# COMBINE-lab/salmon

Hardware: NVIDIA H100
Metric: EM iters/s (higher is better)
Workload: dtype f64

## Files before the change

### salmon_b200/csrc/em.cu

```cuda
#include <cooperative_groups.h>
#include <cub/cub.cuh>
#include <float.h>
#include <math.h>
#include <stdarg.h>
#include <string.h>

#include <algorithm>
#include <string>
#include <vector>

#include "common.cuh"
#include "em_internal.h"

#include "em_kernels.cuh"

namespace sb {

static const void* const K_PERSISTENT[2] = {(const void*)k_em_persistent<false>, (const void*)k_em_persistent<true>};
static const void* const K_PERSISTENT_MGPU[2] = {(const void*)k_em_persistent_mgpu<false>,
                                                 (const void*)k_em_persistent_mgpu<true>};
static void (*const K_P1[2])(EmArgs) = {k_em_p1<false>, k_em_p1<true>};
static void (*const K_P2[2])(EmArgs, uint32_t) = {k_em_p2<false>, k_em_p2<true>};
static void (*const K_P2_PARTIAL[2])(EmArgs) = {k_em_p2_partial<false>, k_em_p2_partial<true>};

// ... 473 lines not shown
  if (!c) return;
  cudaSetDevice(c->device);
  cudaDeviceSynchronize();
  for (void* p : c->x_opened) cudaIpcCloseMemHandle(p);
  cudaFree(c->x_block); cudaFree(c->d_peers); cudaFree(c->d_xfail);
  sb_em_comm_destroy(c);
  free_all(c);
  for (int i = 0; i < 4; ++i) cudaEventDestroy(c->ev[i]);
  cudaStreamDestroy(c->stream);
  delete c;
}

extern "C" int sb_em_set_option(sb_em_ctx* c, const char* key, int64_t value) {
  if (!c || !key) { set_error("null argument"); return SB_ERR_INVALID; }
  if (!strcmp(key, "variant")) c->variant = (int)value;
  else if (!strcmp(key, "blocks_per_sm")) { c->blocks_per_sm = (int)value; c->prepared = false; }
  else if (!strcmp(key, "sell_group_cm") || !strcmp(key, "sell_group_tm")) {
    if (value < 32 || value > (1 << 20) || (value & (value - 1))) { set_error("sell_group must be a power of two >= 32"); return SB_ERR_INVALID; }
    (key[11] == 'c' ? c->sell_group_cm : c->sell_group_tm) = (int)value; c->prepared = false;
  }
  else if (!strcmp(key, "push_pass")) { c->push_pass = (int)value; }
  else if (!strcmp(key, "sample_offset")) { c->sample_offset = (uint32_t)value; }
  else if (!strcmp(key, "rebalance")) { c->rebalance = (int)value; c->prepared = false; }
  else { set_error("unknown option '%s'", key); return SB_ERR_INVALID; }
  return SB_OK;
}

extern "C" int sb_em_get_info(sb_em_ctx* c, const char* key, int64_t* value) {
  if (!c || !key || !value) { set_error("null argument"); return SB_ERR_INVALID; }
  if (!c->prepared) { set_error("sb_em_get_info before sb_em_prepare"); return SB_ERR_STATE; }
  auto stream = [](const SellDev& m) { return (int64_t)m.n_cols * 32 * 10 + (int64_t)m.long_entries * 12; };
  if (!strcmp(key, "stream_bytes")) { *value = stream(c->cm) + stream(c->tm); return SB_OK; }
  if (!strcmp(key, "warps")) { *value = (int64_t)c->grid * (EM_THREADS / 32); return SB_OK; }
  if (!strcmp(key, "ring_cols")) { *value = (int64_t)EM_CH * EM_RING; return SB_OK; }
  const size_t n = strlen(key);
  const SellDev* m = nullptr;
  if (n > 3 && !strcmp(key + n - 3, "_cm")) m = &c->cm;
  else if (n > 3 && !strcmp(key + n - 3, "_tm")) m = &c->tm;
  const std::string k(key, m ? n - 3 : n);
  if (m && k == "stream_bytes") *value = stream(*m);
  else if (m && k == "sell_cols") *value = m->n_cols;
  else if (m && k == "long_rows") *value = m->n_long;
  else if (m && k == "long_entries") *value = (int64_t)m->long_entries;
  else if (m && k == "fallback_rows") *value = m->n_fallback;
  else { set_error("unknown info key '%s'", key); return SB_ERR_INVALID; }
  return SB_OK;
}

extern "C" int sb_em_upload(sb_em_ctx* c, const sb_eq_csr* eq, const double* projected,
                            const double* eff_len, const uint64_t* unique) {
  if (!c || !eq || !projected || !eff_len || !unique) { set_error("null argument"); return SB_ERR_INVALID; }
  if (eq->n_classes && (!eq->off || !eq->counts)) { set_error("null CSR arrays"); return SB_ERR_INVALID; }
  SB_CUDA(cudaSetDevice(c->device));
  const uint64_t C = eq->n_classes;
  const uint32_t M = eq->n_txps;
  const uint64_t nnz = C ? eq->off[C] : 0;
  if (M == 0) { set_error("no transcripts"); return SB_ERR_INVALID; }
  if (nnz >= 0xfffffff0ull || C >= 0xfffffff0ull) {
    set_error("eq-class table too large for 32-bit device offsets (nnz=%llu)", (unsigned long long)nnz);
    return SB_ERR_INVALID;
  }
  if (nnz && (!eq->tids || !eq->weights)) { set_error("null CSR arrays"); return SB_ERR_INVALID; }
  c->C = C; c->M = M; c->nnz = nnz;
  c->prepared = false;
  SB_TRY(dev_alloc(&c->d_off, C + 1));
  SB_TRY(dev_alloc(&c->d_tids, nnz));
  SB_TRY(dev_alloc(&c->d_aux, nnz));
// ... 113 lines not shown
    });
    for (uint32_t i = 0; i < m.n_long; ++i) {
      if (h[3 * ord[i] + 2] - h[3 * ord[i] + 1] > LWARP) m.n_block = i + 1;
      m.long_entries += h[3 * i + 2] - h[3 * i + 1];
    }
    std::vector<uint32_t> h2(h.size());
    for (uint32_t i = 0; i < m.n_long; ++i)
      for (int k = 0; k < 3; ++k) h2[3 * i + k] = h[3 * ord[i] + k];
    SB_CUDA(cudaMemcpyAsync(m.long_rows, h2.data(), h2.size() * 4, cudaMemcpyHostToDevice, st));
    SB_CUDA(cudaStreamSynchronize(st));
  }
  k_warp_ranges<<<nblk(n_warps + 1, 256), 256, 0, st>>>(m.n_slices, m.slice_ptr, overhead, n_warps, m.warp_begin);
  c->launches++;
  return SB_OK;
}

static int em_rebalance(sb_em_ctx* c);

extern "C" int sb_em_prepare(sb_em_ctx* c, const sb_em_params* p, sb_em_stats* stats) {
  if (!c || !p) { set_error("null argument"); return SB_ERR_INVALID; }
  if (!c->uploaded) { set_error("sb_em_prepare before sb_em_upload"); return SB_ERR_STATE; }
  SB_CUDA(cudaSetDevice(c->device));
  cudaStream_t st = c->stream;
  c->params = *p;
  c->launches = 0;
  const uint64_t C = c->C;
  const uint32_t M = c->M;
  const uint64_t nnz = c->nnz;
  const bool row_space = c->nranks <= 1 && !c->fused_loopback;
  SB_CUDA(cudaEventRecord(c->ev[0], st));

  int occ = 0;
  for (int v = 0; v < 2; ++v) {
    SB_CUDA(cudaFuncSetAttribute(K_PERSISTENT[v], cudaFuncAttributeMaxDynamicSharedMemorySize, (int)EM_SMEM));
    SB_CUDA(cudaFuncSetAttribute((const void*)K_P1[v], cudaFuncAttributeMaxDynamicSharedMemorySize, (int)EM_SMEM));
    SB_CUDA(cudaFuncSetAttribute((const void*)K_P2[v], cudaFuncAttributeMaxDynamicSharedMemorySize, (int)EM_SMEM));
    SB_CUDA(cudaFuncSetAttribute((const void*)K_P2_PARTIAL[v], cudaFuncAttributeMaxDynamicSharedMemorySize, (int)EM_SMEM));
    SB_CUDA(cudaFuncSetAttribute(K_PERSISTENT_MGPU[v], cudaFuncAttributeMaxDynamicSharedMemorySize, (int)EM_SMEM));
  }
  const int vb = p->use_vbem ? 1 : 0;
  SB_CUDA(cudaOccupancyMaxActiveBlocksPerMultiprocessor(&occ, (c->nranks > 1 || c->fused_loopback) ? K_PERSISTENT_MGPU[vb] : K_PERSISTENT[vb],
                                                        EM_THREADS, EM_SMEM));
  if (occ < 1) { set_error("persistent EM kernel does not fit on an SM"); return SB_ERR_CUDA; }
  if (c->blocks_per_sm > 0) occ = std::min(occ, c->blocks_per_sm);
  c->grid = (uint32_t)(occ * c->n_sm);
  c->occ = occ;
  const uint32_t n_warps = c->grid * (EM_THREADS / 32);

  const uint64_t NP = std::max<uint64_t>(C, M) + 1;
  const uint64_t NS = std::max<uint64_t>(std::max<uint64_t>(C, nnz), (uint64_t)M) + 1;
  SB_TRY(dev_alloc(&c->d_efflens, M));
  SB_TRY(dev_alloc(&c->d_prior, M));
  SB_TRY(dev_alloc(&c->d_alpha0, M));
  SB_TRY(dev_alloc(&c->d_alpha, M));
  SB_TRY(dev_alloc(&c->d_theta, (size_t)M + 4));
  SB_CUDA(cudaMemsetAsync(c->d_theta, 0, ((size_t)M + 4) * 8, st));
  SB_TRY(dev_alloc(&c->d_base, M));
  SB_TRY(dev_alloc(&c->d_cw, nnz));
  SB_TRY(dev_alloc(&c->d_packed, NP));
  SB_TRY(dev_alloc(&c->d_packed2, NP));
  SB_TRY(dev_alloc(&c->d_packed_scan, NP));
  SB_TRY(dev_alloc(&c->d_valid, C));
  SB_TRY(dev_alloc(&c->d_cls_map, C));
  SB_TRY(dev_alloc(&c->d_scalars, 64));
  SB_TRY(dev_alloc(&c->d_tcnt, M));
  SB_TRY(dev_alloc(&c->d_tid_row, M));
  SB_TRY(dev_alloc(&c->d_sort_keys, NS));
  SB_TRY(dev_alloc(&c->d_sort_vals, NS));
  SB_TRY(dev_alloc(&c->d_sort_keys2, NS));
  SB_TRY(dev_alloc(&c->d_sort_vals2, NS));
  SB_TRY(dev_alloc(&c->d_order, NS));
  SB_CUDA(cudaMemsetAsync(c->d_base, 0, (size_t)M * 8, st));
  SB_CUDA(cudaMemsetAsync(c->d_scalars, 0, 64 * 8, st));
  SB_CUDA(cudaMemsetAsync(c->d_tcnt, 0, (size_t)M * 4, st));
  SB_CUDA(cudaMemsetAsync(c->d_tid_row, 0xff, (size_t)M * 4, st));
// ... 85 lines not shown
  SB_CUDA(cudaMemsetAsync(c->r_theta, 0, ((size_t)R + 4) * 8, st));
  SB_TRY(dev_alloc(&c->r_prior, (size_t)R + 1));
  SB_TRY(dev_alloc(&c->r_base, (size_t)R + 1));
  SB_TRY(dev_alloc(&c->r_alpha0, (size_t)R + 1));
  SB_CUDA(cudaMemcpyAsync(c->t_off + R, &nnzm, 4, cudaMemcpyHostToDevice, st));
  k_rank_fill<<<nblk(M, 256), 256, 0, st>>>(M, c->d_tcnt, c->d_packed_scan, c->t_off, c->d_rank_tid,
                                             c->d_packed2);
  c->launches++;
  if (nnzm) {
    k_gather_csc<<<nblk(nnzm, 256), 256, 0, st>>>(nnzm, c->d_sort_vals2, c->d_ent_cls, c->m_w,
                                                   c->t_idx, c->t_w);
    c->launches++;
  }
  if (R) {
    k_bucket_key<<<nblk(R, 256), 256, 0, st>>>(R, nullptr, c->d_packed2, (uint32_t)c->sell_group_tm, c->d_sort_keys, c->d_sort_vals);
    c->launches++;
    SB_TRY(sort_pairs(c, R, 32));
    SB_CUDA(cudaMemcpyAsync(c->d_rowperm, c->d_sort_vals2, (size_t)R * 4, cudaMemcpyDeviceToDevice, st));
    k_row_fill<<<nblk(R, 256), 256, 0, st>>>(R, c->d_rowperm, c->d_rank_tid, c->d_prior, c->d_base,
                                              c->d_alpha0, c->d_row_tid, c->d_tid_row, c->r_prior,
                                              c->r_base, c->r_alpha0);
    c->launches++;
  }
  if (nnzm) {
    if (row_space) {
      k_remap<<<nblk(nnzm, 256), 256, 0, st>>>(nnzm, c->m_idx, c->d_tid_row, c->m_idx_state);
      c->launches++;
    } else {
      SB_CUDA(cudaMemcpyAsync(c->m_idx_state, c->m_idx, (size_t)nnzm * 4, cudaMemcpyDeviceToDevice, st));
    }
  }
  SB_TRY(build_sell(c, c->cm, Cm, nullptr, c->m_off, c->m_idx_state, c->m_w, row_space ? R : M, OVERHEAD_P1, n_warps));
  SB_TRY(build_sell(c, c->tm, R, c->d_rowperm, c->t_off, c->t_idx, c->t_w, Cm, overhead_tm(c), n_warps));

  double* d_sum0 = c->d_scalars + 16;
  double* d_inact = c->d_scalars + 17;
  k_sum1<<<1, 1024, 0, st>>>(M, c->d_alpha0, c->d_prior, c->d_tid_row, 0, d_sum0);
  k_sum1<<<1, 1024, 0, st>>>(M, c->d_base, c->d_prior, c->d_tid_row, 1, d_inact);
  c->launches += 2;
  SB_CUDA(cudaMemcpyAsync(&c->sum0, d_sum0, 8, cudaMemcpyDeviceToHost, st));
  SB_CUDA(cudaMemcpyAsync(&c->inactive_sum, d_inact, 8, cudaMemcpyDeviceToHost, st));
  SB_TRY(dev_alloc(&c->d_sum_partial, (size_t)2 * std::max<uint32_t>(c->grid, 4096)));
  SB_CUDA(cudaStreamSynchronize(st));
  c->prepared = true;
  c->rebalance_rounds_done = 0;
  if (c->variant == 1 && (c->nranks <= 1 || (c->peers_ready && c->M <= c->x_cap)) && p->max_iter > 0) {
    for (int r = 0; r < c->rebalance; ++r) {
      int rc = em_rebalance(c);
      if (rc != SB_OK) { c->prepared = false; return rc; }
          c->rebalance_rounds_done++;
    }
  }
  const uint32_t prep_launches = c->launches;
  SB_CUDA(cudaEventRecord(c->ev[1], st));
  SB_CUDA(cudaEventSynchronize(c->ev[1]));
  float ms = 0;
  cudaEventElapsedTime(&ms, c->ev[0], c->ev[1]);
  c->prepare_ms = ms;
  c->prepared = true;
  if (stats) {
    memset(stats, 0, sizeof(*stats));
    stats->n_degenerate = c->n_degenerate;
    stats->n_multi_classes = Cm;
    stats->nnz_multi = nnzm;
    stats->n_active_txps = R;
    stats->prepare_ms = ms;
    stats->gpu_launches = prep_launches;
  }
  return SB_OK;
}

static Sell sell_view(const SellDev& m) {
  Sell s;
  s.slice_ptr = m.slice_ptr; s.base = m.base; s.len = m.len; s.idx = m.idx; s.w = m.w; s.warp_begin = m.warp_begin;
  s.long_rows = m.long_rows; s.csr_idx = m.csr_idx; s.csr_w = m.csr_w;
  s.n_rows = m.n_rows; s.n_slices = m.n_slices; s.n_long = m.n_long;
  s.n_block = m.n_block;
  s.zero = m.zero;
  return s;
}

static void fill_args(sb_em_ctx* c, EmArgs& A, bool row_space) {
  memset(&A, 0, sizeof(A));
  A.cm = sell_view(c->cm);
  A.tm = sell_view(c->tm);
  const bool ov = c->ov_active;
  A.c_cnt = (ov && c->ov_cnt) ? c->ov_cnt : c->d_cnt; A.scale = c->d_scale;
  if (row_space) {
    A.alpha = c->r_alpha; A.theta = c->r_theta; A.prior = c->r_prior;
    A.base = (ov && c->ov_base_row) ? c->ov_base_row : c->r_base;
    A.row_tid = nullptr;
  } else {
    A.alpha = c->d_alpha; A.theta = c->d_theta; A.prior = c->d_prior; A.base = c->d_base;
    A.row_tid = c->d_row_tid;
    A.tid_row = c->d_tid_row;
  }
  A.sum_partial = c->d_sum_partial;
  A.maxrel = (unsigned long long*)(c->d_scalars + 24);
  A.inactive_sum = ov ? c->ov_inactive_sum : c->inactive_sum;
  A.sum0 = ov ? c->ov_sum0 : c->sum0;
  A.min_eq_w = ov ? c->ov_min_eq_w : DBL_MIN;
  A.first_bias = ov ? 0.0 : (c->params.use_vbem ? 0.0 : 1.0);
  A.tol = c->params.tol; A.min_iter = c->params.min_iter; A.max_iter = c->params.max_iter;
  A.out = (uint32_t*)(c->d_scalars + 32);
  A.lq = (unsigned int*)(c->d_scalars + 44);
  A.dbg = c->dbg_enabled ? c->d_dbg : nullptr;
  A.dbg_it = c->dbg_it;
}

#include <dlfcn.h>
namespace {
struct NcclUid { char b[128]; };
struct NcclFns {
  void* h = nullptr;
  int (*GetUniqueId)(void*) = nullptr;
  int (*CommInitRank)(void**, int, NcclUid, int) = nullptr;
  int (*AllReduce)(const void*, void*, size_t, int, int, void*, cudaStream_t) = nullptr;
  int (*AllGather)(const void*, void*, size_t, int, void*, cudaStream_t) = nullptr;
  int (*CommDestroy)(void*) = nullptr;
  const char* (*GetErrorString)(int) = nullptr;
};
NcclFns g_nccl;
int nccl_load() {
  if (g_nccl.h) return SB_OK;
  const char* names[] = {"libnccl.so.2", "libnccl.so", nullptr};
  void* h = nullptr;
  for (int i = 0; names[i] && !h; ++i) h = dlopen(names[i], RTLD_NOW | RTLD_GLOBAL);
  if (!h) { set_error("cannot dlopen libnccl.so.2: %s", dlerror()); return SB_ERR_NCCL; }
  g_nccl.GetUniqueId = (decltype(g_nccl.GetUniqueId))dlsym(h, "ncclGetUniqueId");
  g_nccl.CommInitRank = (decltype(g_nccl.CommInitRank))dlsym(h, "ncclCommInitRank");
  g_nccl.AllReduce = (decltype(g_nccl.AllReduce))dlsym(h, "ncclAllReduce");
  g_nccl.AllGather = (decltype(g_nccl.AllGather))dlsym(h, "ncclAllGather");
  g_nccl.CommDestroy = (decltype(g_nccl.CommDestroy))dlsym(h, "ncclCommDestroy");
  g_nccl.GetErrorString = (decltype(g_nccl.GetErrorString))dlsym(h, "ncclGetErrorString");
  if (!g_nccl.GetUniqueId || !g_nccl.CommInitRank || !g_nccl.AllReduce || !g_nccl.AllGather || !g_nccl.CommDestroy) {
    set_error("libnccl is missing required symbols");
    return SB_ERR_NCCL;
  }
  g_nccl.h = h;
  return SB_OK;
// ... 244 lines not shown
  const int vb = c->params.use_vbem ? 1 : 0;
  uint32_t launches = 0;
  SB_CUDA(cudaEventRecord(c->ev[0], st));
  double* d_sum0 = c->d_scalars + 16;
  const bool fused = multi_gpu && c->peers_ready && c->M <= c->x_cap && c->variant == 1;
  const bool ov = c->ov_active;
  if (multi_gpu) {
    double* theta0 = fused ? reinterpret_cast<double*>(c->x_block + XchgLayout(M, (uint32_t)c->nranks).off_theta()) : c->d_theta;
    k_theta0<<<nblk(M, 256), 256, 0, st>>>(M, c->params.use_vbem, c->d_alpha0, c->d_prior, d_sum0,
                                            c->d_alpha, theta0);
    ++launches;
  } else if (R) {
    k_theta0<<<nblk(R, 256), 256, 0, st>>>(R, c->params.use_vbem,
                                            (ov && c->ov_alpha0_row) ? c->ov_alpha0_row : c->r_alpha0,
                                            c->r_prior, ov ? c->d_scalars + 18 : d_sum0,
                                            c->r_alpha, c->r_theta);
    ++launches;
  }
  SB_CUDA(cudaMemsetAsync(c->d_scalars + 24, 0, 16 * 8, st));
  SB_CUDA(cudaMemsetAsync(c->d_scalars + 44, 0, 16, st));
  EmArgs A;
  fill_args(c, A, !multi_gpu);
  uint32_t out[4] = {0, 0, 0, 0};
  float loop_ms = 0;
  uint32_t loop_launches = 0;
  if (c->params.max_iter == 0 && c->params.min_iter == 0) {
  } else if (multi_gpu) {
    int r = fused ? em_run_multi_gpu_fused(c, A, out, &launches, &loop_launches, &loop_ms)
                  : em_run_multi_gpu(c, A, out, &launches, &loop_launches, &loop_ms);
    if (r != SB_OK) return r;
  } else if (c->variant == 1) {
    void* args[] = {(void*)&A};
    SB_CUDA(cudaEventRecord(c->ev[2], st));
    SB_CUDA(cudaLaunchCooperativeKernel(K_PERSISTENT[vb], dim3(c->grid), dim3(EM_THREADS), args, EM_SMEM, st));
    SB_CUDA(cudaEventRecord(c->ev[3], st));
    ++launches; ++loop_launches;
    SB_CUDA(cudaMemcpyAsync(out, A.out, 16, cudaMemcpyDeviceToHost, st));
    SB_CUDA(cudaStreamSynchronize(st));
    cudaEventElapsedTime(&loop_ms, c->ev[2], c->ev[3]);
  } else {
    uint32_t it = 0;
    bool converged = false;
    SB_CUDA(cudaEventRecord(c->ev[2], st));
    while (it < A.min_iter || (it < A.max_iter && !converged)) {
      k_reset_maxrel<<<1, 1, 0, st>>>(A.maxrel, it & 1u);
      K_P1[vb]<<<c->grid, EM_THREADS, EM_SMEM, st>>>(A);
      K_P2[vb]<<<c->grid, EM_THREADS, EM_SMEM, st>>>(A, it);
      launches += 3; loop_launches += 2;
      ++it;
      if (it >= A.min_iter) {
        unsigned long long mr = 0;
        SB_CUDA(cudaMemcpyAsync(&mr, A.maxrel + ((it - 1) & 1u), 8, cudaMemcpyDeviceToHost, st));
        SB_CUDA(cudaStreamSynchronize(st));
        double d;
        memcpy(&d, &mr, 8);
        converged = !(d > A.tol);
      }
    }
    SB_CUDA(cudaEventRecord(c->ev[3], st));
    SB_CUDA(cudaStreamSynchronize(st));
    cudaEventElapsedTime(&loop_ms, c->ev[2], c->ev[3]);
    out[0] = it; out[1] = converged; out[2] = (it - 1) & 1u;
  }
  c->iters = out[0];
  c->converged = out[1];
  if (out[0] > 0) {
    unsigned long long mr = 0;
// ... 185 lines not shown
```

### salmon_b200/csrc/em_internal.h

```cpp
#pragma once
#include <cuda_runtime.h>
#include <stdint.h>

#include <vector>

#include "../../include/salmon_b200.h"

namespace sb {

constexpr int SELL_GROUP = 1024;

struct SellDev {
  uint32_t n_rows = 0, n_slices = 0, n_cols = 0, n_long = 0, n_block = 0;
  uint32_t n_fallback = 0;
  uint64_t long_entries = 0;
  uint32_t zero = 0;
  uint32_t* slice_ptr = nullptr;
  uint32_t* width = nullptr;
  uint32_t* base = nullptr;
  uint16_t* len = nullptr;
  uint16_t* idx = nullptr;
  double* w = nullptr;
  uint32_t* warp_begin = nullptr;
  uint32_t* long_rows = nullptr;
  const uint32_t* csr_idx = nullptr;
  const double* csr_w = nullptr;
};

}

struct sb_em_ctx {
  int device = 0;
  int n_sm = 0;
  size_t l2_bytes = 0;
  cudaStream_t stream = nullptr;
  cudaEvent_t ev[4] = {nullptr, nullptr, nullptr, nullptr};

  int variant = 1;
  int blocks_per_sm = 0;
  int rebalance = 1;
  int occ = 0;
  int sell_group_cm = sb::SELL_GROUP, sell_group_tm = sb::SELL_GROUP;

  uint64_t C = 0, nnz = 0;
  uint32_t M = 0;
  double total_weight = 0.0;
  size_t h2d_bytes = 0;
  bool uploaded = false, prepared = false;
  sb_em_params params{};

  uint64_t* d_off = nullptr;
  uint32_t* d_tids = nullptr;
  double* d_aux = nullptr;
  uint64_t* d_counts = nullptr;
  double* d_projected = nullptr;
  double* d_eff_in = nullptr;
  uint64_t* d_unique = nullptr;

  double* d_efflens = nullptr;
  double* d_prior = nullptr;
  double* d_alpha0 = nullptr;
  double* d_alpha = nullptr;
  double* d_theta = nullptr;
  double* d_base = nullptr;
  uint32_t* d_tcnt = nullptr;
  uint32_t* d_tid_row = nullptr;
  uint32_t* d_row_tid = nullptr;
  double *r_alpha = nullptr, *r_theta = nullptr, *r_prior = nullptr, *r_base = nullptr,
         *r_alpha0 = nullptr;

  double* d_cw = nullptr;
  uint64_t* d_packed = nullptr;
  uint64_t* d_packed2 = nullptr;
  uint64_t* d_packed_scan = nullptr;
// ... 67 lines not shown
```

### salmon_b200/csrc/em_kernels.cuh

```cuda
#pragma once
#include <cooperative_groups.h>
#include <float.h>

#include "common.cuh"
#include "em_math.h"

namespace sb {
namespace cg = cooperative_groups;

constexpr uint32_t LMAX = 96;
constexpr uint32_t LWARP = 2048;
constexpr int EM_THREADS = 256;
constexpr int EM_CH = 8;
constexpr int EM_RING = 4;
constexpr int EM_MIN_BLOCKS = 2;
constexpr double DIGAMMA_MIN = 1e-10;
constexpr double MIN_EQ_W = DBL_MIN;
constexpr double ALPHA_CHECK_CUTOFF = 1e-2;
constexpr uint16_t LEN_LONG = 0xFFFFu;
constexpr uint16_t IDX_PAD = 0xFFFFu;
constexpr uint32_t DBG_ACCUMULATE = 0xFFFFFFFFu;
constexpr uint32_t DBG_SLOTS = 16;

struct Sell {
  const uint32_t* slice_ptr;
  const uint32_t* base;
  const uint16_t* len;
  const uint16_t* idx;
  const double* w;
  const uint32_t* warp_begin;
  const uint32_t* long_rows;
  const uint32_t* csr_idx;
  const double* csr_w;
  uint32_t n_rows, n_slices, n_long;
  uint32_t n_block;
  uint32_t zero;
};

struct EmArgs {
  Sell cm;
  Sell tm;
  const double* c_cnt;
  double* scale;
  double* alpha; double* theta; const double* prior; const double* base;
  const uint32_t* row_tid;
  const uint32_t* tid_row;
  double* part_out;
  double* sum_partial;
  unsigned long long* maxrel;
  double inactive_sum; double sum0;
  double tol;
  double min_eq_w;
  double first_bias;
  uint32_t min_iter, max_iter;
  uint32_t* out;
  unsigned long long* dbg;
  uint32_t dbg_it;
  unsigned int* lq;
  unsigned char* const* peers;
  uint32_t rank, nranks, M;
  uint32_t push_pass;
  unsigned long long epoch0;
  uint32_t* xfail;
};

constexpr uint32_t XAUX = 1024;
struct XchgLayout {
  uint32_t M, G, S;
  __host__ __device__ XchgLayout(uint32_t m, uint32_t g) : M(m), G(g), S((m + g - 1) / g) {}
// ... 3 lines not shown
  __host__ __device__ size_t off_llth() const { return (off_alpha() + (size_t)M * 8 + 15) & ~(size_t)15; }
  __host__ __device__ size_t off_llaux() const { return off_llth() + (size_t)M * 16; }
  __host__ __device__ size_t off_llrecv() const { return off_llaux() + (size_t)G * XAUX * 2 * 16; }
  __host__ __device__ size_t bytes() const { return off_llrecv() + (size_t)G * S * 16; }
};

__device__ __forceinline__ unsigned long long gtime_ns() {
  unsigned long long t;
  asm volatile("mov.u64 %0, %%globaltimer;" : "=l"(t));
  return t;
}

constexpr double SUM_FIXED = 1048576.0;
struct P2Acc {
  long long isum;
  double maxrel;
};
__device__ __forceinline__ long long warp_sum_ll(long long v) {
#pragma unroll
  for (int o = 16; o > 0; o >>= 1) v += __shfl_xor_sync(0xffffffffu, v, o);
  return v;
}
__device__ __forceinline__ long long block_sum_ll(long long v, double* scratch) {
  const int lane = threadIdx.x & 31, wid = threadIdx.x >> 5;
  const int nw = (blockDim.x + 31) >> 5;
  v = warp_sum_ll(v);
  __syncthreads();
  if (lane == 0) scratch[wid] = __longlong_as_double(v);
  __syncthreads();
  long long r = (lane < nw) ? __double_as_longlong(scratch[lane]) : 0ll;
  return warp_sum_ll(r);
}

struct __align__(128) WarpRing {
  double w[EM_RING][EM_CH * 32];
  uint16_t idx[EM_RING][EM_CH * 32];
};
constexpr int EM_WARPS = EM_THREADS / 32;
constexpr size_t EM_SMEM = sizeof(WarpRing) * EM_WARPS + EM_WARPS * EM_RING * 8 + 40 * 8;

struct WarpCtx {
  WarpRing* ring;
  uint64_t* bars;
  uint32_t phase_bits;
  double* scratch;
  uint64_t pol_stream;
  unsigned long long* dbg;
  unsigned long long* dbg_acc;
  unsigned long long t0;
};

__device__ __forceinline__ void warp_setup(WarpCtx& W, unsigned char* smem) {
  const uint32_t wid = threadIdx.x >> 5;
  W.ring = reinterpret_cast<WarpRing*>(smem) + wid;
  W.bars = reinterpret_cast<uint64_t*>(smem + sizeof(WarpRing) * EM_WARPS) + wid * EM_RING;
  W.scratch = reinterpret_cast<double*>(smem + sizeof(WarpRing) * EM_WARPS + EM_WARPS * EM_RING * 8);
  W.phase_bits = 0;
  W.dbg = nullptr;
  W.dbg_acc = nullptr;
  W.t0 = 0;
  W.pol_stream = l2_policy_evict_first();
  if ((threadIdx.x & 31u) == 0) {
#pragma unroll
    for (int s = 0; s < EM_RING; ++s) mbar_init(&W.bars[s], 1);
    mbar_fence_init();
  }
  __syncthreads();
}

struct RowOps {
  double x0, x1, x2, x3;
  uint32_t len;
};
template <int PHASE>
__device__ __forceinline__ RowOps load_ops(const EmArgs& A, const Sell& S, uint32_t row) {
  RowOps o;
  o.x0 = o.x1 = o.x2 = o.x3 = 0.0;
  o.len = LEN_LONG;
  if (row < S.n_rows) {
    o.len = __ldg(&S.len[row]);
    if (PHASE == 1) {
      o.x0 = __ldg(&A.c_cnt[row]);
    } else if (PHASE == 2) {
      o.x0 = A.theta[row];
      o.x1 = __ldg(&A.prior[row]);
      o.x2 = __ldg(&A.base[row]);
      o.x3 = A.alpha[row];
    } else {
      const uint32_t t = __ldg(&A.row_tid[row]);
      o.x0 = A.theta[t];
      o.x2 = __ldg(&A.base[t]);
      o.x3 = __longlong_as_double((long long)t);
    }
  }
  return o;
}

template <bool VBEM>
__device__ __forceinline__ double theta_of(double na, double ap, double logNorm) {
  if (VBEM) return (ap > DIGAMMA_MIN) ? exp_digamma_shifted(ap, logNorm) : 0.0;
  return na;
}

template <int PHASE, bool VBEM, class Deliver>
__device__ __forceinline__ void row_finish(const EmArgs& A, uint32_t row, const RowOps& o, double acc,
                                           double logNorm, double bias, P2Acc& pa, Deliver&& deliver) {
  if (o.len == LEN_LONG) return;
  if (PHASE == 1) {
    A.scale[row] = (acc <= A.min_eq_w) ? 0.0 : o.x0 / acc;
  } else if (PHASE == 2) {
    const double th = o.x0, pr = o.x1;
    double na = o.x2 + bias;
    if (th > 0.0) na = fma(th, acc, na);
    if (na > ALPHA_CHECK_CUTOFF) pa.maxrel = fmax(pa.maxrel, fabs(o.x3 - na) / na);
    A.alpha[row] = na;
    const double ap = na + pr;
    pa.isum += __double2ll_rn(ap * SUM_FIXED);
    A.theta[row] = theta_of<VBEM>(na, ap, logNorm);
  } else {
    const uint32_t t = (uint32_t)__double_as_longlong(o.x3);
    double na = o.x2;
    if (o.x0 > 0.0) na = fma(o.x0, acc, na);
    deliver(t, na);
  }
}

struct WarpRange {
  uint32_t s0, s1, cbeg, cend;
};
__device__ __forceinline__ WarpRange load_range(const Sell& S, uint32_t gwarp) {
  WarpRange r;
  r.s0 = __ldg(&S.warp_begin[gwarp]);
  r.s1 = __ldg(&S.warp_begin[gwarp + 1]);
  r.cbeg = __ldg(&S.slice_ptr[r.s0]);
  r.cend = __ldg(&S.slice_ptr[r.s1]);
  return r;
}
__device__ __forceinline__ void ring_issue(const Sell& S, WarpCtx& W, const WarpRange& R, uint32_t k) {
  if ((threadIdx.x & 31u) == 0) {
    const uint32_t c = R.cbeg + k * EM_CH;
    const uint32_t cols = min((uint32_t)EM_CH, R.cend - c);
    const int st = k % EM_RING;
    mbar_arrive_expect_tx(&W.bars[st], cols * 320u);
    bulk_g2s_hint(W.ring->w[st], S.w + (size_t)c * 32u, cols * 256u, &W.bars[st], W.pol_stream);
    bulk_g2s_hint(W.ring->idx[st], S.idx + (size_t)c * 32u, cols * 64u, &W.bars[st], W.pol_stream);
  }
}
__device__ __forceinline__ void ring_prefetch(const Sell& S, WarpCtx& W, const WarpRange& R) {
  const uint32_t nchunks = (R.cend - R.cbeg + EM_CH - 1) / EM_CH;
#pragma unroll
  for (int k = 0; k < EM_RING; ++k)
    if ((uint32_t)k < nchunks) ring_issue(S, W, R, k);
}
__device__ __forceinline__ void ring_drain(WarpCtx& W, const WarpRange& R) {
  const uint32_t nchunks = (R.cend - R.cbeg + EM_CH - 1) / EM_CH;
#pragma unroll
  for (int k = 0; k < EM_RING; ++k)
    if ((uint32_t)k < nchunks) mbar_wait(&W.bars[k], (W.phase_bits >> k) & 1u);
}

struct RingCols {
  static constexpr uint32_t RC = (uint32_t)(EM_CH * EM_RING);
  const Sell& S;
  WarpCtx& W;
  const WarpRange& R;
  uint32_t lane, nchunks;
  uint32_t done = 0, ready = 0;
  __device__ __forceinline__ void need(uint32_t c0, uint32_t c1) {
    for (; (done + 1u) * EM_CH <= c0; ++done) {
      __syncwarp();
      if (done + EM_RING < nchunks) ring_issue(S, W, R, done + EM_RING);
    }
    for (; ready * EM_CH < c1; ++ready) {
      const int st = ready % EM_RING;
      mbar_wait(&W.bars[st], (W.phase_bits >> st) & 1u);
      W.phase_bits ^= (1u << st);
    }
  }
  __device__ __forceinline__ uint32_t group_at(uint32_t c) const {
    const uint32_t p = (c % RC) * 32u + lane * 4u;
    return p >= RC * 32u ? p - RC * 32u : p;
  }
  __device__ __forceinline__ uint2 idx4(uint32_t c) const {
    return *reinterpret_cast<const uint2*>(&W.ring->idx[0][0] + group_at(c));
  }
  __device__ __forceinline__ double2 w4(uint32_t c, uint32_t j) const {
    return *reinterpret_cast<const double2*>(&W.ring->w[0][0] + group_at(c) + j);
  }
  __device__ __forceinline__ uint32_t idx1(uint32_t c) const { return (&W.ring->idx[0][0])[(c % RC) * 32u + lane]; }
  __device__ __forceinline__ double w1(uint32_t c) const { return (&W.ring->w[0][0])[(c % RC) * 32u + lane]; }
};
template <int PHASE, bool VBEM, class Deliver>
__device__ __forceinline__ void sell_rows(const EmArgs& A, const Sell& S, RingCols& cols, uint32_t s0,
                                          uint32_t s1, uint32_t cbeg, uint32_t cend, double logNorm, double bias,
                                          P2Acc& pa, Deliver&& deliver) {
  const double* gsrc = (PHASE == 1) ? A.theta : A.scale;
  constexpr bool GUARD = (PHASE == 1) && !VBEM;
  const uint32_t lane = threadIdx.x & 31u;
  auto slot = [&](uint32_t base, uint32_t u) { return u == IDX_PAD ? S.zero : base + u; };
  auto fma1 = [&](double& acc, double g, double w) {
    if (GUARD) {
      const double v = g * w;
      if (!isnan(v)) acc += v;
    } else {
      acc = fma(g, w, acc);
    }
  };
  struct Group {
    double g0, g1, g2, g3;
    double2 wa, wb;
  };
  auto group_load = [&](uint32_t c, uint32_t base) {
    const uint2 i2 = cols.idx4(c);
    Group q;
    q.g0 = gsrc[slot(base, i2.x & 0xFFFFu)];
    q.g1 = gsrc[slot(base, i2.x >> 16)];
    q.g2 = gsrc[slot(base, i2.y & 0xFFFFu)];
    q.g3 = gsrc[slot(base, i2.y >> 16)];
    q.wa = cols.w4(c, 0u);
    q.wb = cols.w4(c, 2u);
    return q;
  };
  auto group_fma = [&](double& acc, const Group& q) {
    fma1(acc, q.g0, q.wa.x); fma1(acc, q.g1, q.wa.y); fma1(acc, q.g2, q.wb.x); fma1(acc, q.g3, q.wb.y);
  };
  uint32_t sbase = s0;
// ... 19 lines not shown
      cols.need(c, c + 8);
      const Group qa = group_load(c, base);
      const Group qb = group_load(c + 4, base);
      group_fma(acc, qa);
      group_fma(acc, qb);
    }
    if (ng) {
      cols.need(c, c + 4);
      group_fma(acc, group_load(c, base));
      c += 4;
    }
    if (rem) {
      cols.need(c, c + rem);
      const double g0 = gsrc[slot(base, cols.idx1(c))];
      if (rem == 1) {
        fma1(acc, g0, cols.w1(c));
      } else if (rem == 2) {
        const double g1 = gsrc[slot(base, cols.idx1(c + 1))];
        fma1(acc, g0, cols.w1(c)); fma1(acc, g1, cols.w1(c + 1));
      } else {
        const double g1 = gsrc[slot(base, cols.idx1(c + 1))], g2 = gsrc[slot(base, cols.idx1(c + 2))];
        fma1(acc, g0, cols.w1(c)); fma1(acc, g1, cols.w1(c + 1)); fma1(acc, g2, cols.w1(c + 2));
      }
      c += rem;
    }
    row_finish<PHASE, VBEM>(A, s * 32u + lane, ops, acc, logNorm, bias, pa, deliver);
  }
}

struct Nothing {
  __device__ __forceinline__ void operator()() const {}
};

template <int PHASE, bool VBEM, bool DYNQ, class AfterHome, class Deliver>
__device__ __forceinline__ void run_phase(const EmArgs& A, WarpCtx& W, const WarpRange& R,
                                          uint32_t bid, uint32_t nblk, double logNorm, double bias,
                                          P2Acc& pa, AfterHome&& after_home, Deliver&& deliver) {
  static_assert(EM_CH >= 8 && EM_RING >= 2, "two groups in flight span at most two resident chunks");
  const Sell& S = (PHASE == 1) ? A.cm : A.tm;
  const double* gsrc = (PHASE == 1) ? A.theta : A.scale;
  constexpr bool GUARD = (PHASE == 1) && !VBEM;
  const uint32_t lane = threadIdx.x & 31u;
  if (R.s1 > R.s0 && R.cend > R.cbeg) {
    RingCols rc{S, W, R, lane, (R.cend - R.cbeg + EM_CH - 1) / EM_CH};
    sell_rows<PHASE, VBEM>(A, S, rc, R.s0, R.s1, R.cbeg, R.cend, logNorm, bias, pa, deliver);
  }
  unsigned long long* const dbg = W.dbg;
  if (dbg && lane == 0) dbg[PHASE == 1 ? 8 : 7] = gtime_ns();
  if (W.dbg_acc && lane == 0) *W.dbg_acc += gtime_ns() - W.t0;
  __syncwarp();
  after_home();
  for (uint32_t li = bid; li < S.n_block; li += nblk) {
    const uint32_t r = __ldg(&S.long_rows[3 * li]);
    const uint32_t b = __ldg(&S.long_rows[3 * li + 1]);
    const uint32_t e = __ldg(&S.long_rows[3 * li + 2]);
    double a0 = 0.0, a1 = 0.0;
    uint32_t k = b + threadIdx.x;
    for (; k + EM_THREADS < e; k += 2 * EM_THREADS) {
      const uint32_t i0 = __ldg(&S.csr_idx[k]), i1 = __ldg(&S.csr_idx[k + EM_THREADS]);
      double v0 = gsrc[i0] * __ldg(&S.csr_w[k]);
      double v1 = gsrc[i1] * __ldg(&S.csr_w[k + EM_THREADS]);
      if (GUARD) {
        if (isnan(v0)) v0 = 0.0;
        if (isnan(v1)) v1 = 0.0;
      }
      a0 += v0;
      a1 += v1;
    }
    if (k < e) {
      double v = gsrc[__ldg(&S.csr_idx[k])] * __ldg(&S.csr_w[k]);
      if (GUARD && isnan(v)) v = 0.0;
      a0 += v;
    }
    const double acc = block_reduce<false>(a0 + a1, W.scratch);
    if (threadIdx.x == 0) {
      RowOps o = load_ops<PHASE>(A, S, r);
      o.len = 0;
      row_finish<PHASE, VBEM>(A, r, o, acc, logNorm, bias, pa, deliver);
// ... 102 lines not shown
__device__ __forceinline__ void lag_lognorm_warp0(const EmArgs& A, uint32_t par, uint32_t nblk,
                                                  double* scratch) {
  if (threadIdx.x < 32) {
    const double* part = A.sum_partial + (size_t)(par ^ 1u) * nblk;
    long long acc = 0;
    for (uint32_t i = threadIdx.x; i < nblk; i += 32) acc += __double_as_longlong(__ldcg(&part[i]));
    acc = warp_sum_ll(acc);
    if (threadIdx.x == 0) scratch[33] = digamma_pos((double)acc / SUM_FIXED + A.inactive_sum);
  }
}

__device__ __forceinline__ void p2_finish(const EmArgs& A, double* scratch, P2Acc& pa,
                                          uint32_t par) {
  const long long bs = block_sum_ll(pa.isum, scratch);
  double bm = block_reduce<true>(pa.maxrel, scratch);
  if (threadIdx.x == 0) {
    A.sum_partial[(size_t)par * gridDim.x + blockIdx.x] = __longlong_as_double(bs);
    if (bm > 0.0) atomicMax(&A.maxrel[par], (unsigned long long)__double_as_longlong(bm));
  }
}

#define SB_DBG(slot)                                                        \
  if (A.dbg && it == A.dbg_it && (threadIdx.x & 31u) == 0) A.dbg[(size_t)gwarp * DBG_SLOTS + (slot)] = gtime_ns();
#define SB_ACC_BEGIN(var, sell_slot) \
  unsigned long long var = 0; \
  if (dbg_acc) { var = gtime_ns(); W.t0 = var; W.dbg_acc = &A.dbg[(size_t)gwarp * DBG_SLOTS + (sell_slot)]; }
#define SB_ACC_END(var, slot) \
  W.dbg_acc = nullptr; \
  if (dbg_acc && (threadIdx.x & 31u) == 0) A.dbg[(size_t)gwarp * DBG_SLOTS + (slot)] += gtime_ns() - var;

template <bool VBEM>
__global__ void __launch_bounds__(EM_THREADS, EM_MIN_BLOCKS) k_em_persistent(const __grid_constant__ EmArgs A) {
  extern __shared__ __align__(128) unsigned char smem[];
  WarpCtx W;
  warp_setup(W, smem);
  double* scratch = W.scratch;
  cg::grid_group grid = cg::this_grid();
  const uint32_t bid = blockIdx.x, nblk = gridDim.x;
  const uint32_t gwarp = bid * (EM_THREADS / 32) + (threadIdx.x >> 5);
  const WarpRange R1 = load_range(A.cm, gwarp);
  const WarpRange R2 = load_range(A.tm, gwarp);
  uint32_t it = 0;
  bool converged = false;
  double logNorm = VBEM ? digamma_pos(A.sum0) : 0.0;
  ring_prefetch(A.cm, W, R1);
  while (it < A.min_iter || (it < A.max_iter && !converged)) {
    const uint32_t par = it & 1u;
    const bool dbg_acc = A.dbg && A.dbg_it == DBG_ACCUMULATE && it > 0;
    if (bid == 0 && threadIdx.x == 0) A.maxrel[par] = 0ull;
    if (VBEM && it > 0) lag_lognorm_warp0(A, par, nblk, scratch);
    P2Acc pa{0ll, 0.0};
    SB_DBG(0)
    SB_ACC_BEGIN(t1, 3)
    W.dbg = (A.dbg && it == A.dbg_it) ? &A.dbg[(size_t)gwarp * DBG_SLOTS] : nullptr;
    run_phase<1, VBEM, true>(A, W, R1, bid, nblk, 0.0, 0.0, pa, [&] { ring_prefetch(A.tm, W, R2); }, NoDeliver{});
    SB_ACC_END(t1, 0)
    SB_DBG(1)
    grid.sync();
    SB_DBG(2)
    if (bid == 0 && threadIdx.x == 0) A.lq[0] = 0u;
    if (VBEM && it > 0) logNorm = scratch[33];
    const double bias = (it == 0) ? A.first_bias : 0.0;
    SB_DBG(3)
    SB_ACC_BEGIN(t2, 4)
    run_phase<2, VBEM, true>(A, W, R2, bid, nblk, logNorm, bias, pa, [&] { ring_prefetch(A.cm, W, R1); }, NoDeliver{});
    W.dbg = nullptr;
    SB_ACC_END(t2, 1)
    SB_DBG(4)
    p2_finish(A, scratch, pa, par);
    SB_DBG(5)
    grid.sync();
    SB_DBG(6)
    if (bid == 0 && threadIdx.x == 0) A.lq[1] = 0u;
    if (dbg_acc && (threadIdx.x & 31u) == 0) A.dbg[(size_t)gwarp * DBG_SLOTS + 2] += 1ull;
// ... 291 lines not shown
```

Baseline: 26620.

## Keep leading SELL slices resident in shared memory across EM iterations

The persistent EM kernel now reserves spare shared memory per warp and, once at kernel start, bulk-loads the first SELL columns of each warp's cm and tm ranges into it. Each iteration then processes those slices straight from shared memory, and only the remaining columns are streamed through a smaller ring buffer (3 stages instead of 4). This is meant to cut repeated global/L2 streaming of matrix data on every iteration, at the cost of a shallower prefetch ring and more shared memory per block, which is capped to keep two blocks per SM. An info query for resident bytes is also added.

New measurement: 27180, median of 6. +2.1%, better.

```diff
diff --git a/salmon_b200/csrc/em.cu b/salmon_b200/csrc/em.cu
--- a/salmon_b200/csrc/em.cu
+++ b/salmon_b200/csrc/em.cu
@@ -529,7 +529,36 @@
   auto stream = [](const SellDev& m) { return (int64_t)m.n_cols * 32 * 10 + (int64_t)m.long_entries * 12; };
   if (!strcmp(key, "stream_bytes")) { *value = stream(c->cm) + stream(c->tm); return SB_OK; }
   if (!strcmp(key, "warps")) { *value = (int64_t)c->grid * (EM_THREADS / 32); return SB_OK; }
-  if (!strcmp(key, "ring_cols")) { *value = (int64_t)EM_CH * EM_RING; return SB_OK; }
+  if (!strcmp(key, "ring_cols")) { *value = (int64_t)EM_CH * EM_RING_RES; return SB_OK; }
+  if (!strcmp(key, "resident_cols_cm")) { *value = c->res_cm; return SB_OK; }
+  if (!strcmp(key, "resident_cols_tm")) { *value = c->res_cm ? EM_RES_COLS : 0; return SB_OK; }
+  if (!strcmp(key, "resident_bytes")) {
+    if (c->res_cm == 0) { *value = 0; return SB_OK; }
+    const uint32_t n_warps = c->grid * (EM_THREADS / 32);
+    std::vector<uint32_t> sp[2], wb[2];
+    SB_CUDA(cudaSetDevice(c->device));
+    for (int l = 0; l < 2; ++l) {
+      const SellDev& m = l ? c->tm : c->cm;
+      sp[l].resize((size_t)m.n_slices + 1);
+      wb[l].resize((size_t)n_warps + 1);
+      SB_CUDA(cudaMemcpy(sp[l].data(), m.slice_ptr, sp[l].size() * 4, cudaMemcpyDeviceToHost));
+      SB_CUDA(cudaMemcpy(wb[l].data(), m.warp_begin, wb[l].size() * 4, cudaMemcpyDeviceToHost));
+    }
+    int64_t b = 0;
+    for (uint32_t w = 0; w < n_warps; ++w) {
+      uint32_t budget = c->res_cm;
+      for (int l = 0; l < 2; ++l) {
+        const uint32_t s0 = wb[l][w], s1 = wb[l][w + 1];
+        uint32_t k = 0;
+        while (k < 32 && s0 + k < s1 && sp[l][s0 + k + 1] - sp[l][s0] <= budget) ++k;
+        const uint32_t cols = sp[l][s0 + k] - sp[l][s0];
+        b += (int64_t)cols * 320;
+        budget = EM_RES_COLS - cols;
+      }
+    }
+    *value = b;
+    return SB_OK;
+  }
   const size_t n = strlen(key);
   const SellDev* m = nullptr;
   if (n > 3 && !strcmp(key + n - 3, "_cm")) m = &c->cm;
@@ -709,15 +738,16 @@
 
   int occ = 0;
   for (int v = 0; v < 2; ++v) {
-    SB_CUDA(cudaFuncSetAttribute(K_PERSISTENT[v], cudaFuncAttributeMaxDynamicSharedMemorySize, (int)EM_SMEM));
+    SB_CUDA(cudaFuncSetAttribute(K_PERSISTENT[v], cudaFuncAttributeMaxDynamicSharedMemorySize, (int)EM_SMEM_RES));
     SB_CUDA(cudaFuncSetAttribute((const void*)K_P1[v], cudaFuncAttributeMaxDynamicSharedMemorySize, (int)EM_SMEM));
     SB_CUDA(cudaFuncSetAttribute((const void*)K_P2[v], cudaFuncAttributeMaxDynamicSharedMemorySize, (int)EM_SMEM));
     SB_CUDA(cudaFuncSetAttribute((const void*)K_P2_PARTIAL[v], cudaFuncAttributeMaxDynamicSharedMemorySize, (int)EM_SMEM));
     SB_CUDA(cudaFuncSetAttribute(K_PERSISTENT_MGPU[v], cudaFuncAttributeMaxDynamicSharedMemorySize, (int)EM_SMEM));
   }
   const int vb = p->use_vbem ? 1 : 0;
-  SB_CUDA(cudaOccupancyMaxActiveBlocksPerMultiprocessor(&occ, (c->nranks > 1 || c->fused_loopback) ? K_PERSISTENT_MGPU[vb] : K_PERSISTENT[vb],
-                                                        EM_THREADS, EM_SMEM));
+  const bool mgpu_kernel = c->nranks > 1 || c->fused_loopback;
+  SB_CUDA(cudaOccupancyMaxActiveBlocksPerMultiprocessor(&occ, mgpu_kernel ? K_PERSISTENT_MGPU[vb] : K_PERSISTENT[vb],
+                                                        EM_THREADS, mgpu_kernel ? EM_SMEM : EM_SMEM_RES));
   if (occ < 1) { set_error("persistent EM kernel does not fit on an SM"); return SB_ERR_CUDA; }
   if (c->blocks_per_sm > 0) occ = std::min(occ, c->blocks_per_sm);
   c->grid = (uint32_t)(occ * c->n_sm);
@@ -869,6 +899,7 @@
   }
   SB_TRY(build_sell(c, c->cm, Cm, nullptr, c->m_off, c->m_idx_state, c->m_w, row_space ? R : M, OVERHEAD_P1, n_warps));
   SB_TRY(build_sell(c, c->tm, R, c->d_rowperm, c->t_off, c->t_idx, c->t_w, Cm, overhead_tm(c), n_warps));
+  c->res_cm = row_space ? EM_RES_COLS : 0u;
 
   double* d_sum0 = c->d_scalars + 16;
   double* d_inact = c->d_scalars + 17;
@@ -914,6 +945,7 @@
   s.n_rows = m.n_rows; s.n_slices = m.n_slices; s.n_long = m.n_long;
   s.n_block = m.n_block;
   s.zero = m.zero;
+  s.nres = 0;
   return s;
 }
 
@@ -943,6 +975,7 @@
   A.lq = (unsigned int*)(c->d_scalars + 44);
   A.dbg = c->dbg_enabled ? c->d_dbg : nullptr;
   A.dbg_it = c->dbg_it;
+  A.cm.nres = c->res_cm;
 }
 
 #include <dlfcn.h>
@@ -1253,7 +1286,7 @@
   } else if (c->variant == 1) {
     void* args[] = {(void*)&A};
     SB_CUDA(cudaEventRecord(c->ev[2], st));
-    SB_CUDA(cudaLaunchCooperativeKernel(K_PERSISTENT[vb], dim3(c->grid), dim3(EM_THREADS), args, EM_SMEM, st));
+    SB_CUDA(cudaLaunchCooperativeKernel(K_PERSISTENT[vb], dim3(c->grid), dim3(EM_THREADS), args, EM_SMEM_RES, st));
     SB_CUDA(cudaEventRecord(c->ev[3], st));
     ++launches; ++loop_launches;
     SB_CUDA(cudaMemcpyAsync(out, A.out, 16, cudaMemcpyDeviceToHost, st));
diff --git a/salmon_b200/csrc/em_internal.h b/salmon_b200/csrc/em_internal.h
--- a/salmon_b200/csrc/em_internal.h
+++ b/salmon_b200/csrc/em_internal.h
@@ -40,6 +40,7 @@
   int blocks_per_sm = 0;
   int rebalance = 1;
   int occ = 0;
+  uint32_t res_cm = 0;
   int sell_group_cm = sb::SELL_GROUP, sell_group_tm = sb::SELL_GROUP;
 
   uint64_t C = 0, nnz = 0;
diff --git a/salmon_b200/csrc/em_kernels.cuh b/salmon_b200/csrc/em_kernels.cuh
--- a/salmon_b200/csrc/em_kernels.cuh
+++ b/salmon_b200/csrc/em_kernels.cuh
@@ -14,6 +14,8 @@
 constexpr int EM_CH = 8;
 constexpr int EM_RING = 4;
 constexpr int EM_MIN_BLOCKS = 2;
+constexpr int EM_RING_RES = 3;
+constexpr size_t EM_SMEM_MAX = 115712;
 constexpr double DIGAMMA_MIN = 1e-10;
 constexpr double MIN_EQ_W = DBL_MIN;
 constexpr double ALPHA_CHECK_CUTOFF = 1e-2;
@@ -35,6 +37,7 @@
   uint32_t n_rows, n_slices, n_long;
   uint32_t n_block;
   uint32_t zero;
+  uint32_t nres;
 };
 
 struct EmArgs {
@@ -104,15 +107,23 @@
   return warp_sum_ll(r);
 }
 
-struct __align__(128) WarpRing {
-  double w[EM_RING][EM_CH * 32];
-  uint16_t idx[EM_RING][EM_CH * 32];
+template <int NR>
+struct __align__(128) WarpRingT {
+  double w[NR][EM_CH * 32];
+  uint16_t idx[NR][EM_CH * 32];
 };
 constexpr int EM_WARPS = EM_THREADS / 32;
-constexpr size_t EM_SMEM = sizeof(WarpRing) * EM_WARPS + EM_WARPS * EM_RING * 8 + 40 * 8;
-
-struct WarpCtx {
-  WarpRing* ring;
+template <int NR>
+constexpr size_t ring_smem() { return sizeof(WarpRingT<NR>) * EM_WARPS + EM_WARPS * NR * 8 + 40 * 8; }
+constexpr size_t EM_SMEM = ring_smem<EM_RING>();
+constexpr size_t EM_SMEM_RING_RES = ring_smem<EM_RING_RES>();
+constexpr uint32_t EM_RES_COLS = (uint32_t)((EM_SMEM_MAX - EM_SMEM_RING_RES - EM_WARPS * 8) / (EM_WARPS * 320));
+constexpr size_t EM_SMEM_RES = EM_SMEM_RING_RES + EM_WARPS * 8 + (size_t)EM_WARPS * EM_RES_COLS * 320;
+static_assert(EM_SMEM_RES <= EM_SMEM_MAX, "k_em_persistent must keep EM_MIN_BLOCKS blocks per SM");
+
+template <int NR>
+struct WarpCtxT {
+  WarpRingT<NR>* ring;
   uint64_t* bars;
   uint32_t phase_bits;
   double* scratch;
@@ -121,12 +132,14 @@
   unsigned long long* dbg_acc;
   unsigned long long t0;
 };
-
-__device__ __forceinline__ void warp_setup(WarpCtx& W, unsigned char* smem) {
+using WarpCtx = WarpCtxT<EM_RING>;
+
+template <int NR>
+__device__ __forceinline__ void warp_setup(WarpCtxT<NR>& W, unsigned char* smem) {
   const uint32_t wid = threadIdx.x >> 5;
-  W.ring = reinterpret_cast<WarpRing*>(smem) + wid;
-  W.bars = reinterpret_cast<uint64_t*>(smem + sizeof(WarpRing) * EM_WARPS) + wid * EM_RING;
-  W.scratch = reinterpret_cast<double*>(smem + sizeof(WarpRing) * EM_WARPS + EM_WARPS * EM_RING * 8);
+  W.ring = reinterpret_cast<WarpRingT<NR>*>(smem) + wid;
+  W.bars = reinterpret_cast<uint64_t*>(smem + sizeof(WarpRingT<NR>) * EM_WARPS) + wid * NR;
+  W.scratch = reinterpret_cast<double*>(smem + sizeof(WarpRingT<NR>) * EM_WARPS + EM_WARPS * NR * 8);
   W.phase_bits = 0;
   W.dbg = nullptr;
   W.dbg_acc = nullptr;
@@ -134,7 +147,7 @@
   W.pol_stream = l2_policy_evict_first();
   if ((threadIdx.x & 31u) == 0) {
 #pragma unroll
-    for (int s = 0; s < EM_RING; ++s) mbar_init(&W.bars[s], 1);
+    for (int s = 0; s < NR; ++s) mbar_init(&W.bars[s], 1);
     mbar_fence_init();
   }
   __syncthreads();
@@ -198,7 +211,9 @@
 }
 
 struct WarpRange {
+  static constexpr bool RESIDENT = false;
   uint32_t s0, s1, cbeg, cend;
+  __device__ __forceinline__ uint32_t sbeg() const { return cbeg; }
 };
 __device__ __forceinline__ WarpRange load_range(const Sell& S, uint32_t gwarp) {
   WarpRange r;
@@ -208,43 +223,91 @@
   r.cend = __ldg(&S.slice_ptr[r.s1]);
   return r;
 }
-__device__ __forceinline__ void ring_issue(const Sell& S, WarpCtx& W, const WarpRange& R, uint32_t k) {
+struct ResRange : WarpRange {
+  static constexpr bool RESIDENT = true;
+  uint32_t sres, nres;
+  const double* rw;
+  const uint16_t* ri;
+  __device__ __forceinline__ uint32_t sbeg() const { return cbeg + nres; }
+};
+__device__ __forceinline__ ResRange load_res_range(const Sell& S, uint32_t gwarp, uint32_t ncols, uint32_t off,
+                                                   unsigned char* smem) {
+  ResRange r;
+  static_cast<WarpRange&>(r) = load_range(S, gwarp);
+  const uint32_t lane = threadIdx.x & 31u;
+  const bool in = r.s0 + lane < r.s1;
+  const uint32_t end = in ? __ldg(&S.slice_ptr[r.s0 + lane + 1u]) : r.cend;
+  const uint32_t k = __popc(__ballot_sync(0xffffffffu, in && end - r.cbeg <= ncols));
+  r.sres = r.s0 + k;
+  r.nres = k ? __shfl_sync(0xffffffffu, end, (int)k - 1) - r.cbeg : 0u;
+  unsigned char* area = smem + EM_SMEM_RING_RES + EM_WARPS * 8 + (threadIdx.x >> 5) * (EM_RES_COLS * 320u);
+  r.rw = reinterpret_cast<const double*>(area) + off * 32u;
+  r.ri = reinterpret_cast<const uint16_t*>(area + EM_RES_COLS * 256u) + off * 32u;
+  return r;
+}
+__device__ __forceinline__ void res_load(const Sell& S1, const ResRange& R1, const Sell& S2, const ResRange& R2,
+                                         uint64_t pol, unsigned char* smem) {
+  uint64_t* bar = reinterpret_cast<uint64_t*>(smem + EM_SMEM_RING_RES) + (threadIdx.x >> 5);
+  const uint32_t bytes = (R1.nres + R2.nres) * 320u;
+  if (bytes == 0) return;
   if ((threadIdx.x & 31u) == 0) {
-    const uint32_t c = R.cbeg + k * EM_CH;
+    mbar_init(bar, 1);
+    mbar_fence_init();
+    mbar_arrive_expect_tx(bar, bytes);
+    if (R1.nres) {
+      bulk_g2s_hint(const_cast<double*>(R1.rw), S1.w + (size_t)R1.cbeg * 32u, R1.nres * 256u, bar, pol);
+      bulk_g2s_hint(const_cast<uint16_t*>(R1.ri), S1.idx + (size_t)R1.cbeg * 32u, R1.nres * 64u, bar, pol);
+    }
+    if (R2.nres) {
+      bulk_g2s_hint(const_cast<double*>(R2.rw), S2.w + (size_t)R2.cbeg * 32u, R2.nres * 256u, bar, pol);
+      bulk_g2s_hint(const_cast<uint16_t*>(R2.ri), S2.idx + (size_t)R2.cbeg * 32u, R2.nres * 64u, bar, pol);
+    }
+  }
+  __syncwarp();
+  mbar_wait(bar, 0u);
+}
+
+template <int NR, class Range>
+__device__ __forceinline__ void ring_issue(const Sell& S, WarpCtxT<NR>& W, const Range& R, uint32_t k) {
+  if ((threadIdx.x & 31u) == 0) {
+    const uint32_t c = R.sbeg() + k * EM_CH;
     const uint32_t cols = min((uint32_t)EM_CH, R.cend - c);
-    const int st = k % EM_RING;
+    const int st = k % NR;
     mbar_arrive_expect_tx(&W.bars[st], cols * 320u);
     bulk_g2s_hint(W.ring->w[st], S.w + (size_t)c * 32u, cols * 256u, &W.bars[st], W.pol_stream);
     bulk_g2s_hint(W.ring->idx[st], S.idx + (size_t)c * 32u, cols * 64u, &W.bars[st], W.pol_stream);
   }
 }
-__device__ __forceinline__ void ring_prefetch(const Sell& S, WarpCtx& W, const WarpRange& R) {
-  const uint32_t nchunks = (R.cend - R.cbeg + EM_CH - 1) / EM_CH;
+template <int NR, class Range>
+__device__ __forceinline__ void ring_prefetch(const Sell& S, WarpCtxT<NR>& W, const Range& R) {
+  const uint32_t nchunks = (R.cend - R.sbeg() + EM_CH - 1) / EM_CH;
 #pragma unroll
-  for (int k = 0; k < EM_RING; ++k)
+  for (int k = 0; k < NR; ++k)
     if ((uint32_t)k < nchunks) ring_issue(S, W, R, k);
 }
-__device__ __forceinline__ void ring_drain(WarpCtx& W, const WarpRange& R) {
-  const uint32_t nchunks = (R.cend - R.cbeg + EM_CH - 1) / EM_CH;
+template <int NR, class Range>
+__device__ __forceinline__ void ring_drain(WarpCtxT<NR>& W, const Range& R) {
+  const uint32_t nchunks = (R.cend - R.sbeg() + EM_CH - 1) / EM_CH;
 #pragma unroll
-  for (int k = 0; k < EM_RING; ++k)
+  for (int k = 0; k < NR; ++k)
     if ((uint32_t)k < nchunks) mbar_wait(&W.bars[k], (W.phase_bits >> k) & 1u);
 }
 
+template <int NR, class Range>
 struct RingCols {
-  static constexpr uint32_t RC = (uint32_t)(EM_CH * EM_RING);
+  static constexpr uint32_t RC = (uint32_t)(EM_CH * NR);
   const Sell& S;
-  WarpCtx& W;
-  const WarpRange& R;
+  WarpCtxT<NR>& W;
+  const Range& R;
   uint32_t lane, nchunks;
   uint32_t done = 0, ready = 0;
   __device__ __forceinline__ void need(uint32_t c0, uint32_t c1) {
     for (; (done + 1u) * EM_CH <= c0; ++done) {
       __syncwarp();
-      if (done + EM_RING < nchunks) ring_issue(S, W, R, done + EM_RING);
+      if (done + NR < nchunks) ring_issue(S, W, R, done + NR);
     }
     for (; ready * EM_CH < c1; ++ready) {
-      const int st = ready % EM_RING;
+      const int st = ready % NR;
       mbar_wait(&W.bars[st], (W.phase_bits >> st) & 1u);
       W.phase_bits ^= (1u << st);
     }
@@ -262,8 +325,22 @@
   __device__ __forceinline__ uint32_t idx1(uint32_t c) const { return (&W.ring->idx[0][0])[(c % RC) * 32u + lane]; }
   __device__ __forceinline__ double w1(uint32_t c) const { return (&W.ring->w[0][0])[(c % RC) * 32u + lane]; }
 };
-template <int PHASE, bool VBEM, class Deliver>
-__device__ __forceinline__ void sell_rows(const EmArgs& A, const Sell& S, RingCols& cols, uint32_t s0,
+struct ResCols {
+  const double* w;
+  const uint16_t* idx;
+  uint32_t lane;
+  __device__ __forceinline__ void need(uint32_t, uint32_t) const {}
+  __device__ __forceinline__ uint2 idx4(uint32_t c) const {
+    return *reinterpret_cast<const uint2*>(idx + c * 32u + lane * 4u);
+  }
+  __device__ __forceinline__ double2 w4(uint32_t c, uint32_t j) const {
+    return *reinterpret_cast<const double2*>(w + c * 32u + lane * 4u + j);
+  }
+  __device__ __forceinline__ uint32_t idx1(uint32_t c) const { return idx[c * 32u + lane]; }
+  __device__ __forceinline__ double w1(uint32_t c) const { return w[c * 32u + lane]; }
+};
+template <int PHASE, bool VBEM, class Cols, class Deliver>
+__device__ __forceinline__ void sell_rows(const EmArgs& A, const Sell& S, Cols& cols, uint32_t s0,
                                           uint32_t s1, uint32_t cbeg, uint32_t cend, double logNorm, double bias,
                                           P2Acc& pa, Deliver&& deliver) {
   const double* gsrc = (PHASE == 1) ? A.theta : A.scale;
@@ -349,18 +426,28 @@
   __device__ __forceinline__ void operator()() const {}
 };
 
-template <int PHASE, bool VBEM, bool DYNQ, class AfterHome, class Deliver>
-__device__ __forceinline__ void run_phase(const EmArgs& A, WarpCtx& W, const WarpRange& R,
+template <int PHASE, bool VBEM, bool DYNQ, int NR, class Range, class AfterHome, class Deliver>
+__device__ __forceinline__ void run_phase(const EmArgs& A, WarpCtxT<NR>& W, const Range& R,
                                           uint32_t bid, uint32_t nblk, double logNorm, double bias,
                                           P2Acc& pa, AfterHome&& after_home, Deliver&& deliver) {
-  static_assert(EM_CH >= 8 && EM_RING >= 2, "two groups in flight span at most two resident chunks");
+  static_assert(EM_CH >= 8 && NR >= 2, "two groups in flight span at most two resident chunks");
   const Sell& S = (PHASE == 1) ? A.cm : A.tm;
   const double* gsrc = (PHASE == 1) ? A.theta : A.scale;
   constexpr bool GUARD = (PHASE == 1) && !VBEM;
   const uint32_t lane = threadIdx.x & 31u;
   if (R.s1 > R.s0 && R.cend > R.cbeg) {
-    RingCols rc{S, W, R, lane, (R.cend - R.cbeg + EM_CH - 1) / EM_CH};
-    sell_rows<PHASE, VBEM>(A, S, rc, R.s0, R.s1, R.cbeg, R.cend, logNorm, bias, pa, deliver);
+    uint32_t s0 = R.s0;
+    if constexpr (Range::RESIDENT) {
+      if (R.sres > R.s0) {
+        ResCols res{R.rw, R.ri, lane};
+        sell_rows<PHASE, VBEM>(A, S, res, R.s0, R.sres, R.cbeg, R.sbeg(), logNorm, bias, pa, deliver);
+      }
+      s0 = R.sres;
+    }
+    if (R.s1 > s0) {
+      RingCols<NR, Range> rc{S, W, R, lane, (R.cend - R.sbeg() + EM_CH - 1) / EM_CH};
+      sell_rows<PHASE, VBEM>(A, S, rc, s0, R.s1, R.sbeg(), R.cend, logNorm, bias, pa, deliver);
+    }
   }
   unsigned long long* const dbg = W.dbg;
   if (dbg && lane == 0) dbg[PHASE == 1 ? 8 : 7] = gtime_ns();
@@ -529,14 +616,15 @@
 template <bool VBEM>
 __global__ void __launch_bounds__(EM_THREADS, EM_MIN_BLOCKS) k_em_persistent(const __grid_constant__ EmArgs A) {
   extern __shared__ __align__(128) unsigned char smem[];
-  WarpCtx W;
+  WarpCtxT<EM_RING_RES> W;
   warp_setup(W, smem);
   double* scratch = W.scratch;
   cg::grid_group grid = cg::this_grid();
   const uint32_t bid = blockIdx.x, nblk = gridDim.x;
   const uint32_t gwarp = bid * (EM_THREADS / 32) + (threadIdx.x >> 5);
-  const WarpRange R1 = load_range(A.cm, gwarp);
-  const WarpRange R2 = load_range(A.tm, gwarp);
+  const ResRange R1 = load_res_range(A.cm, gwarp, A.cm.nres, 0u, smem);
+  const ResRange R2 = load_res_range(A.tm, gwarp, EM_RES_COLS - R1.nres, R1.nres, smem);
+  res_load(A.cm, R1, A.tm, R2, W.pol_stream, smem);
   uint32_t it = 0;
   bool converged = false;
   double logNorm = VBEM ? digamma_pos(A.sum0) : 0.0;
```
